# hoivb612/neural

Hardware: AMD Instinct MI355X
Metric: decode tokens/sec + prefill TFLOPS, Llama-2-7B int4-g128 at 1/2/4/8 MI355X (higher is better)
Workload: dtype f16; 1 GPU; Llama-2-7B int4-g128 sym decode linear stack, M=1 (32 x [QKV, O, gate/up+SiLU*mul, down] + lm_head), fp32 activations; group_size=128, batch=1, tp=1, parallelism=tp1, hip_graph=True

## Files before the change

neural_amd/csrc/woq_gemv.hip:

```cpp
#include <hip/hip_runtime.h>

#include <climits>
#include <cstdint>
#include <type_traits>

#include "woq_device.h"
#include "woq_kernels.h"

namespace nad {

#ifdef NAD_PHASE_TRACE
constexpr int kTraceSlots = 8, kTraceMaxWg = 16384;
__device__ unsigned long long nad_trace_buf[kTraceSlots][kTraceMaxWg];
#define NAD_TRACE(slot)                                                                       \
  do {                                                                                        \
    if (threadIdx.x == 0 && blockIdx.x < kTraceMaxWg) nad_trace_buf[slot][blockIdx.x] = wall_clock64(); \
  } while (0)
#define NAD_TRACE_MAX(slot)                                                                               \
  do {                                                                                                    \
    if ((threadIdx.x & 63) == 0 && blockIdx.x < kTraceMaxWg)                                              \
      atomicMax(&nad_trace_buf[slot][blockIdx.x], (unsigned long long)wall_clock64());                    \
  } while (0)
#else
#define NAD_TRACE(slot) \
// ... 153 lines not shown

template <int ST>
__device__ __forceinline__ float scale_to_f32(uint32_t x, int st, int sh) {
  if constexpr (ST < 0) return scale_bits_to_f32(x, st, sh);
  else if constexpr (ST == kScaleF32) return __uint_as_float(x);
  else if constexpr (ST == kScaleBF16) return __uint_as_float((x >> sh) << 16);
  else return f16_bits_to_f32(uint16_t(x >> sh));
}

constexpr int k_tile(int bits) { return bits == 4 ? 128 : (bits == 2 ? 256 : 64); }
constexpr int zp_bias(int bits) { return bits == 4 ? 8 : (bits == 2 ? 2 : 128); }

template <int BITS>
__device__ __forceinline__ Dq4 dq4_consts(uint32_t mask, uint32_t magic) {
  Dq4 q;
  q.m0 = __builtin_amdgcn_readfirstlane(mask);
  q.m1 = q.m0 << 4;
  q.mag = __builtin_amdgcn_readfirstlane(magic);
  q.s16 = splat(1.f / 16.f);
  q.c0 = splat(-(1024.f + zp_bias(BITS)));
  q.c1 = splat(-(64.f + zp_bias(BITS)));
  return q;
}

template <int BITS, bool ASYM>
__device__ __forceinline__ h8_t dequant_tile_step(const u4_t& b, int d, int zp, const Dq4& dq) {
  if constexpr (BITS == 4) {
    if constexpr (ASYM) {
      const float z = float(zp);
      return dequant4(b[d], dq, dq.c0 - splat(z), dq.c1 - splat(z));
    } else {
      return dequant4(b[d], dq, dq.c0, dq.c1);
    }
  } else {
    return BITS == 2 ? dequant2_step(b, d, zp_bias(BITS) + zp) : dequant_step<BITS>(b, d, zp_const(zp_bias(BITS) + zp));
  }
}

template <int BITS, int GPT, bool ASYM, int KSN, int ST, bool LO, class TileOff>
__device__ __forceinline__ void stage_mac(const StageRegs<GPT, KSN>& S, const Dq4& dq, const char* ab, const char* abl,
                                          TileOff tile_off, int scale_t, int ssh, f4_t& acc) {
  constexpr int SPT = k_tile(BITS) / 32, SPG = SPT / GPT;
  f4_t accg[KSN];
#pragma unroll
  for (int d = 0; d < SPT; d++) {
    const int g = GPT == 1 ? 0 : d / SPG;
#pragma unroll
    for (int i = 0; i < KSN; i++) {
      const h8_t bf = dequant_tile_step<BITS, ASYM>(S.b[i], d, S.zp[i][g], dq);
      const h8_t af = *reinterpret_cast<const h8_t*>(ab + tile_off(i) + d * 64);
      accg[i] = __builtin_amdgcn_mfma_f32_16x16x32_f16(af, bf, d % SPG == 0 ? f4_t{0.f, 0.f, 0.f, 0.f} : accg[i], 0, 0, 0);
      if constexpr (LO) {
        const h8_t afl = *reinterpret_cast<const h8_t*>(abl + tile_off(i) + d * 64);
        accg[i] = __builtin_amdgcn_mfma_f32_16x16x32_f16(afl, bf, accg[i], 0, 0, 0);
      }
    }
    if ((d + 1) % SPG == 0) {
#pragma unroll
      for (int i = 0; i < KSN; i++) acc += accg[i] * scale_to_f32<ST>(S.sc[i][g], scale_t, ssh);
    }
  }
}

__device__ __forceinline__ float reduce_slots(const float* ps, int nwl) {
  float t[16];
#pragma unroll
  for (int w = 0; w < 16; w++) t[w] = ps[min(w, nwl - 1)];
  const int full = nwl & ~3;
  float s0 = 0.f, s1 = 0.f, s2 = 0.f, s3 = 0.f;
#pragma unroll
  for (int w = 0; w < 16; w += 4)
    if (w < full) {
      s0 += t[w];
      s1 += t[w + 1];
      s2 += t[w + 2];
      s3 += t[w + 3];
    }
#pragma unroll
  for (int w = 0; w < 16; w++)
    if (w >= full && w < nwl) s0 += t[w];
  return (s0 + s1) + (s2 + s3);
}

__device__ __forceinline__ float reduce16(const float* col) {
  const float4* ps = reinterpret_cast<const float4*>(col);
  const float4 t0 = ps[0], t1 = ps[1], t2 = ps[2], t3 = ps[3];
  const float s0 = ((t0.x + t1.x) + t2.x) + t3.x, s1 = ((t0.y + t1.y) + t2.y) + t3.y;
  const float s2 = ((t0.z + t1.z) + t2.z) + t3.z, s3 = ((t0.w + t1.w) + t2.w) + t3.w;
  return (s0 + s1) + (s2 + s3);
}

__device__ __forceinline__ void unit_to_f32(int act_t, uint4 x0, uint4 x1, float (&f)[8]) {
  const uint32_t w[8] = {x0.x, x0.y, x0.z, x0.w, x1.x, x1.y, x1.z, x1.w};
  if (act_t == kActF32) {
#pragma unroll
    for (int j = 0; j < 8; j++) f[j] = __uint_as_float(w[j]);
  } else if (act_t == kActBF16) {
#pragma unroll
    for (int j = 0; j < 4; j++) {
      f[2 * j] = __uint_as_float(w[j] << 16);
      f[2 * j + 1] = __uint_as_float(w[j] & 0xFFFF0000u);
    }
  } else {
#pragma unroll
    for (int j = 0; j < 4; j++) {
      const h2_t h = as_h2(w[j]);
      f[2 * j] = float(h[0]);
      f[2 * j + 1] = float(h[1]);
    }
  }
}

template <int HILO>
__device__ __forceinline__ void unit_store(char* smem, const float (&f)[8], int row, int k, int M, int Kp) {
  h8_t hi, lo;
#pragma unroll
  for (int j = 0; j < 8; j++) {
    hi[j] = _Float16(f[j]);
    lo[j] = _Float16(f[j] - float(hi[j]));
  }
  *reinterpret_cast<h8_t*>(smem + (size_t(row) * Kp + k) * 2) = hi;
  if constexpr (HILO != 0) *reinterpret_cast<h8_t*>(smem + (size_t(M + row) * Kp + k) * 2) = lo;
}

template <int HILO>
__device__ __forceinline__ void stage_a_slow(const GemvArgs& a, char* smem, int units, int Kp) {
  for (int u = threadIdx.x; u < units; u += blockDim.x) {
    const int row = u / (Kp >> 3), k = (u - row * (Kp >> 3)) * 8;
    float f[8];
    for (int j = 0; j < 8; j++) {
      const int kk = k + j;
      f[j] = 0.f;
      if (kk < a.K) {
        const size_t src = size_t(row) * a.lda + (a.shuffle ? a.shuffle[kk] : kk);
        if (a.act_t == kActF32)
          f[j] = static_cast<const float*>(a.A)[src];
        else if (a.act_t == kActBF16)
          f[j] = bf16_bits_to_f32(static_cast<const uint16_t*>(a.A)[src]);
        else
          f[j] = float(static_cast<const _Float16*>(a.A)[src]);
      }
    }
    unit_store<HILO>(smem, f, row, k, a.M, Kp);
  }
}

template <int GPT>
constexpr int gemv_max_threads() {
  return GPT == 1 ? 1024 : 512;
}

template <int BITS, int HILO, int GPT, bool ASYM, int NST>
__global__ __launch_bounds__(gemv_max_threads<GPT>()) void woq_gemv_kernel(GemvArgs a) {
  extern __shared__ __attribute__((aligned(16))) char smem[];
  constexpr int KT = k_tile(BITS);
  static_assert(KT / 32 % GPT == 0, "groups must tile the K tile");
  const int lane = threadIdx.x & 63;
  const int wave = __builtin_amdgcn_readfirstlane(int(threadIdx.x >> 6));
  const int NW = __builtin_amdgcn_readfirstlane(int(blockDim.x >> 6));
  const int M = a.M, nt = a.nt, Kp = nt * KT;
  const int R = HILO == 0 ? M : 2 * M;
  const int nsl = (nt + KS - 1) / KS;
  NAD_TRACE(0);

  const int G = gridDim.x, bid = blockIdx.x;
  const int u0 = int(unsigned(bid) * unsigned(a.units) / unsigned(G));
  const int u1 = int(unsigned(bid + 1) * unsigned(a.units) / unsigned(G));
  const int vpu = a.dual ? 2 : 1;
  const int v0 = u0 * vpu, nv = (u1 - u0) * vpu;
  const bool idle = wave >= nsl;
  float* part = reinterpret_cast<float*>(smem + a.part_off);
// ... 141 lines not shown
    float v = y[0];
    switch (a.epi) {
      case kEpiBias:
        v += a.w[0].bias[size_t(mm) * a.w[0].bias_ld + n];
        break;
      case kEpiAddGelu:
        v = gelu_f(v + a.w[0].bias[size_t(mm) * a.w[0].bias_ld + n]);
        break;
      case kEpiGelu:
        v = gelu_f(v);
        break;
      case kEpiSilu:
        v = silu_f(v);
        break;
      case kEpiResAdd:
        v += a.res[size_t(mm) * a.ld_res + n];
        break;
      case kEpiSiluMul: {
        const float t1 = silu_f(y[0]);
        if (a.aux) a.aux[size_t(mm) * a.ld_aux + n] = t1;
        v = t1 * y[1];
        break;
      }
      case kEpiGeluMul: {
        const float t1 = gelu_f(y[0]);
        if (a.aux) a.aux[size_t(mm) * a.ld_aux + n] = t1;
        v = t1 * y[1];
        break;
      }
      default:
        break;
    }
    out[size_t(mm) * ldo + n] = v;
  }
  NAD_TRACE(3);
}

constexpr int lean_row_bytes(int bits, int ks) { return ks * (bits == 4 ? 128 : 256) * 2; }
constexpr int lean_wave_lds(int bits, int ks, int spw) { return lean_row_bytes(bits, ks) * (1 + 2 * spw); }
static int lean_ks(const GemvArgs& a) { return a.lean_ks == 1 || a.lean_ks == 2 ? a.lean_ks : KS; }
template <int GPT, int KSN>
constexpr int m1_max_threads() {
  return GPT == 1 || KSN <= 2 ? 1024 : 512;
}
static int lean_spw(const GemvArgs& a) { return a.lean_spw == 4 ? 4 : (a.lean_spw == 1 ? 1 : 2); }

static bool lean_ok(const GemvArgs& a, int bits, int waves) {
  int tpg = 0;
  const int ks = lean_ks(a);
  const int nsl = (a.nt + ks - 1) / ks;
  const int gpt = gemv_groups_per_tile(bits, a.nt, a.ng, a.bs, &tpg);
  const bool inst = bits == 4 ? (gpt == 1 || gpt == 2) : (bits == 2 && (gpt == 1 || gpt == 2 || (gpt == 4 && !a.asym)));
  return a.lean && a.M == 1 && inst && a.a_fast && nsl <= waves * lean_spw(a);
}

#ifndef NAD_M1_BATCH_NST
#define NAD_M1_BATCH_NST 3
#endif
#ifndef NAD_M1_DUAL_NST
#define NAD_M1_DUAL_NST 2
#endif

struct M1General {
  using Args = GemvArgs;
  static __device__ __forceinline__ __amdgpu_buffer_rsrc_t act_rsrc(const Args& a, int esz) { return rsrc(a.A, a.K * esz); }
  static __device__ __forceinline__ bool act_live(const Args& a, int q, int nsl, int k) { return q < nsl && k < a.K; }
  template <bool ASYM>
  static __device__ __forceinline__ void cursor_start(const Args& a, StageCursor& c, int v0, int nv, bool idle) {
    c.s = 0;
    c.rt = rsrc(a.w[0].tiles, 0);
    c.rs = c.rt;
    c.rz = c.rt;
    if (!idle && nv > 0) cursor_stripe(a, c, v0);
  }
  template <int GPT, bool ASYM, int KSN>
  static __device__ __forceinline__ void load(const Args& a, StageRegs<GPT, KSN>& S, StageCursor& c, int nv, int nsl,
                                              int wave, int NW, int v0, int lane, int vs) {
    load_stage<GPT, ASYM, KSN>(a, S, c, nv, nsl, wave, NW, v0, lane, vs);
  }
};

template <class P, int BITS, int GPT, int AT, bool ASYM, int KSN, int SPW, int NST, int ST>
__device__ __forceinline__ void m1_stream(const typename P::Args& a, int lane, int wave, int NW, int nsl, int v0,
                                          int nv, bool idle, float* part) {
  extern __shared__ __attribute__((aligned(16))) char smem[];
  constexpr int KT = k_tile(BITS);
  constexpr int RB = lean_row_bytes(BITS, KSN);
  constexpr int UNITS = KSN * KT / 8;
  constexpr int UPL = UNITS >= 64 ? UNITS / 64 : 1;
  constexpr bool PART = UNITS < 64;
  constexpr int ESZ = AT == kActF32 ? 4 : 2;
  constexpr bool HL = AT != kActF16;
  const bool ulane = !PART || lane < UNITS;

  const auto ra = P::act_rsrc(a, ESZ);
  uint4 x[SPW * UPL][2];
#pragma unroll
  for (int j = 0; j < SPW * UPL; j++) {
    const int q = wave + (j / UPL) * NW, k = q * (KSN * KT) + ((j % UPL) * 64 + lane) * 8;
    const int off = (ulane && P::act_live(a, q, nsl, k)) ? k * ESZ : kOOB;
    x[j][0] = __builtin_bit_cast(uint4, __builtin_amdgcn_raw_buffer_load_b128(ra, off, 0, 0));
    if constexpr (ESZ == 4) x[j][1] = __builtin_bit_cast(uint4, __builtin_amdgcn_raw_buffer_load_b128(ra, off + 16, 0, 0));
  }
  const int vs = a.scale_t == kScaleF32 ? (lane & 15) * 4 : (lane & 14) * 2;
  StageCursor lc;
  lc.j = idle ? nv : 0;
  lc.q = wave;
  P::template cursor_start<ASYM>(a, lc, v0, nv, idle);
  StageRegs<GPT, KSN> S[NST];
  P::template load<GPT, ASYM, KSN>(a, S[0], lc, nv, nsl, wave, NW, v0, lane, vs);
  NAD_TRACE(4);

  char* wrow = smem + wave * lean_wave_lds(BITS, KSN, SPW);
#pragma unroll
  for (int u = 0; u < UPL; u++)
    if (ulane) *reinterpret_cast<uint4*>(wrow + (u * 64 + lane) * 16) = make_uint4(0u, 0u, 0u, 0u);
#pragma unroll
  for (int j = 0; j < SPW * UPL; j++) {
    if (!ulane) break;
    h8_t hi, lo;
    if constexpr (AT == kActF16) {
      hi = __builtin_bit_cast(h8_t, x[j][0]);
    } else {
      float f[8];
      unit_to_f32(AT, x[j][0], x[j][1], f);
#pragma unroll
      for (int e = 0; e < 8; e++) {
        hi[e] = _Float16(f[e]);
        lo[e] = _Float16(f[e] - float(hi[e]));
      }
    }
    char* row = wrow + RB + (j / UPL) * 2 * RB + ((j % UPL) * 64 + lane) * 16;
    *reinterpret_cast<h8_t*>(row) = hi;
    if constexpr (HL) *reinterpret_cast<h8_t*>(row + RB) = lo;
  }
#pragma unroll
  for (int i = 1; i < NST; i++) P::template load<GPT, ASYM, KSN>(a, S[i], lc, nv, nsl, wave, NW, v0, lane, vs);
  NAD_TRACE(1);

  const int m = lane & 15, kq = lane >> 4;
  const bool isrow = m == 0 || (HL && m == 8);
  const char* abase = wrow + (isrow ? (m == 0 ? RB : 2 * RB) : 0) + kq * 16;
  const int slice_step = isrow ? 2 * RB : 0;
  const int ssh = a.scale_t == kScaleF32 ? 0 : (lane & 1) * 16;
  const Dq4 dq = dq4_consts<BITS>(a.dq_mask, a.dq_magic);

  f4_t acc = {0.f, 0.f, 0.f, 0.f};
  int cj = idle ? nv : 0, cq = wave, cs = 0;

  auto compute_stage = [&](const StageRegs<GPT, KSN>& S) {
    if (cj >= nv) return;
    const char* ab = abase + cs * slice_step;
    stage_mac<BITS, GPT, ASYM, KSN, ST, false>(S, dq, ab, ab, [](int i) { return i * KT * 2; }, a.scale_t, ssh, acc);
    cq += NW;
    cs++;
    if (cq >= nsl) {
      float r = acc[0];
      if constexpr (HL) {
        r += __shfl_down(r, 32, 64);
      }
      if (lane < 16) part[(size_t(cj) * 16 + lane) * NW + wave] = r;
      acc = f4_t{0.f, 0.f, 0.f, 0.f};
      cq = wave;
      cs = 0;
      cj++;
    }
  };

  while (cj < nv) {
#pragma unroll
    for (int i = 0; i < NST; i++) {
      compute_stage(S[i]);
      P::template load<GPT, ASYM, KSN>(a, S[i], lc, nv, nsl, wave, NW, v0, lane, vs);
    }
  }
  NAD_TRACE_MAX(2);
  __syncthreads();
}

template <int BITS, int GPT, int AT, bool ASYM, int KSN, int SPW, bool BATCH, int NST, int ST = -1>
__device__ __forceinline__ void m1_body(GemvArgs& a, int bid) {
  extern __shared__ __attribute__((aligned(16))) char smem[];
  const int lane = threadIdx.x & 63;
  const int wave = __builtin_amdgcn_readfirstlane(int(threadIdx.x >> 6));
  const int NW = __builtin_amdgcn_readfirstlane(int(blockDim.x >> 6));
  const int nsl = (a.nt + KSN - 1) / KSN;
  NAD_TRACE(0);
  if constexpr (BATCH) {
    const int p = bid / a.batch_wpp;
    bid -= p * a.batch_wpp;
    const GemvBatchEnt e = a.batch[p];
    a.A = e.act;
    a.w[0].tiles = e.tiles;
    a.w[0].scales = e.scales;
    a.w[0].zps = e.zps;
    a.w[0].out = e.out;
  }
  const int u0 = bid * a.u_q + min(bid, a.u_r);
  const int u1 = u0 + a.u_q + (bid < a.u_r ? 1 : 0);
  const int vpu = a.dual ? 2 : 1;
  const int v0 = u0 * vpu, nv = (u1 - u0) * vpu;
  float* part = reinterpret_cast<float*>(smem + a.part_off);
  m1_stream<M1General, BITS, GPT, AT, ASYM, KSN, SPW, NST, ST>(a, lane, wave, NW, nsl, v0, nv, wave >= nsl, part);

  const int nout = (u1 - u0) * 16;
  const int nwl = min(NW, nsl);
  auto emit = [&](int p, int nn, const float (&y)[2]) {
    int wsel, s;
    vstripe(a, v0 + p * vpu, wsel, s);
    if (a.dual) wsel = 0;
    const int n = s * 16 + nn;
    if (n >= sel3(wsel, a.w[0].n, a.w[1].n, a.w[2].n)) return;
    float* out = sel3(wsel, a.w[0].out, a.w[1].out, a.w[2].out);
    float v = y[0];
    switch (a.epi) {
      case kEpiBias:
        v += a.w[0].bias[n];
        break;
      case kEpiAddGelu:
        v = gelu_f(v + a.w[0].bias[n]);
        break;
      case kEpiGelu:
        v = gelu_f(v);
        break;
      case kEpiSilu:
        v = silu_f(v);
        break;
      case kEpiResAdd:
        v += a.res[n];
        break;
      case kEpiSiluMul: {
        const float t1 = silu_f(y[0]);
        if (a.aux) a.aux[n] = t1;
        v = t1 * y[1];
        break;
      }
      case kEpiGeluMul: {
        const float t1 = gelu_f(y[0]);
        if (a.aux) a.aux[n] = t1;
        v = t1 * y[1];
        break;
      }
      default:
        break;
    }
    out[n] = v;
  };
  if (nwl == 16 && NW == 16) {
    for (int o = threadIdx.x; o < nout; o += blockDim.x) {
      const int p = o >> 4, nn = o & 15;
      float y[2] = {0.f, 0.f};
#pragma unroll
      for (int h = 0; h < 2; h++)
        if (h < vpu) y[h] = reduce16(part + (size_t(p * vpu + h) * 16 + nn) * 16);
      emit(p, nn, y);
    }
    NAD_TRACE(3);
    return;
  }
  for (int o = threadIdx.x; o < nout; o += blockDim.x) {
    const int p = o >> 4, nn = o & 15;
    float y[2] = {0.f, 0.f};
#pragma unroll
    for (int h = 0; h < 2; h++)
      if (h < vpu) y[h] = reduce_slots(part + (size_t(p * vpu + h) * 16 + nn) * NW, nwl);
    emit(p, nn, y);
  }
  NAD_TRACE(3);
}

template <int BITS, int GPT, int AT, bool ASYM, int KSN, int SPW, bool BATCH, int NST, int ST>
__global__ __launch_bounds__((m1_max_threads<GPT, KSN>())) void woq_gemv_m1_kernel(GemvArgs a) {
  m1_body<BITS, GPT, AT, ASYM, KSN, SPW, BATCH, NST, ST>(a, int(blockIdx.x));
}

template <int B1, int G1, int K1, int B2, int G2, int K2, int AT>
__global__ __launch_bounds__(1024) void woq_gemv_m1_dual_kernel(GemvArgs a, GemvArgs b, int ga) {
  if (int(blockIdx.x) < ga)
    m1_body<B1, G1, AT, false, K1, 1, false, NAD_M1_DUAL_NST>(a, int(blockIdx.x));
  else
    m1_body<B2, G2, AT, false, K2, 1, false, NAD_M1_DUAL_NST>(b, int(blockIdx.x) - ga);
}

template <int NWT>
struct M1Sel {
  int w, s;
  __device__ __forceinline__ M1Sel(const GemvM1Args<NWT>& a, int v) {
    if constexpr (NWT == 1) {
      w = 0;
      s = v;
    } else if constexpr (NWT == 2) {
      w = v & 1;
      s = v >> 1;
    } else {
      w = (v >= a.sb1 ? 1 : 0) + (v >= a.sb2 ? 1 : 0);
      s = v - (w == 0 ? 0 : (w == 1 ? a.sb1 : a.sb2));
    }
  }
};
template <int NWT, class T>
__device__ __forceinline__ T m1_pick(int w, const T (&x)[3]) {
  if constexpr (NWT == 1) return x[0];
  else if constexpr (NWT == 2) return w == 0 ? x[0] : x[1];
  else return sel3(w, x[0], x[1], x[2]);
}
#define NAD_M1_FIELD(args, wi, f) \
  m1_pick<NWT>(wi, {args.w[0].f, args.w[NWT > 1 ? 1 : 0].f, args.w[NWT > 2 ? 2 : 0].f})

template <int NWT, bool ASYM>
__device__ __forceinline__ void m1s_cursor_stripe(const GemvM1Args<NWT>& a, StageCursor& c, int v, bool on) {
  const M1Sel<NWT> vs(a, v);
  c.s = vs.s;
  const void* const tp[3] = {a.w[0].tiles, a.w[NWT > 1 ? 1 : 0].tiles, a.w[NWT > 2 ? 2 : 0].tiles};
  const void* const sp[3] = {a.w[0].scales, a.w[NWT > 1 ? 1 : 0].scales, a.w[NWT > 2 ? 2 : 0].scales};
  const int tb[3] = {a.w[0].tiles_bytes, a.w[NWT > 1 ? 1 : 0].tiles_bytes, a.w[NWT > 2 ? 2 : 0].tiles_bytes};
  const int sb[3] = {a.w[0].scales_bytes, a.w[NWT > 1 ? 1 : 0].scales_bytes, a.w[NWT > 2 ? 2 : 0].scales_bytes};
  c.rt = rsrc(m1_pick<NWT>(vs.w, tp), on ? m1_pick<NWT>(vs.w, tb) : 0);
  c.rs = rsrc(m1_pick<NWT>(vs.w, sp), on ? m1_pick<NWT>(vs.w, sb) : 0);
  if constexpr (ASYM) {
    const void* const zp[3] = {a.w[0].zps, a.w[NWT > 1 ? 1 : 0].zps, a.w[NWT > 2 ? 2 : 0].zps};
    const int zb[3] = {a.w[0].zps_bytes, a.w[NWT > 1 ? 1 : 0].zps_bytes, a.w[NWT > 2 ? 2 : 0].zps_bytes};
    c.rz = rsrc(m1_pick<NWT>(vs.w, zp), on ? m1_pick<NWT>(vs.w, zb) : 0);
  } else {
    c.rz = c.rs;
  }
}

template <int GPT, bool ASYM, int KSN, int NWT>
__device__ __forceinline__ void m1s_load_stage(const GemvM1Args<NWT>& a, StageRegs<GPT, KSN>& S, StageCursor& c, int nv,
                                               int nsl, int wave, int NW, int v0, int lane, int vs) {
  const bool on = c.j < nv;
  stage_loads<ASYM>(a, S, c, on, lane, vs);
  if (on) {
    c.q += NW;
    if (c.q >= nsl) {
      c.q = wave;
      c.j++;
      m1s_cursor_stripe<NWT, ASYM>(a, c, v0 + c.j, c.j < nv);
    }
  }
}

template <int NWT>
struct M1Spec {
  using Args = GemvM1Args<NWT>;
  static __device__ __forceinline__ __amdgpu_buffer_rsrc_t act_rsrc(const Args& a, int) { return rsrc(a.A, a.a_bytes); }
  static __device__ __forceinline__ bool act_live(const Args&, int, int, int) { return true; }
  template <bool ASYM>
  static __device__ __forceinline__ void cursor_start(const Args& a, StageCursor& c, int v0, int nv, bool) {
    m1s_cursor_stripe<NWT, ASYM>(a, c, v0, c.j < nv);
  }
  template <int GPT, bool ASYM, int KSN>
  static __device__ __forceinline__ void load(const Args& a, StageRegs<GPT, KSN>& S, StageCursor& c, int nv, int nsl,
                                              int wave, int NW, int v0, int lane, int vs) {
    m1s_load_stage<GPT, ASYM, KSN, NWT>(a, S, c, nv, nsl, wave, NW, v0, lane, vs);
  }
};

template <int BITS, int GPT, int AT, bool ASYM, int KSN, int SPW, int NST, int ST, int NWT, bool L16>
__global__ __launch_bounds__((m1_max_threads<GPT, KSN>())) void woq_gemv_m1s_kernel(GemvM1Args<NWT> a) {
  extern __shared__ __attribute__((aligned(16))) char smem[];
  static_assert(NWT >= 1 && NWT <= 3, "1 weight, the {gate, up} pair, or 3 weights");
  constexpr int VPU = NWT == 2 ? 2 : 1;
  const int lane = threadIdx.x & 63;
  const int wave = __builtin_amdgcn_readfirstlane(int(threadIdx.x >> 6));
  const int NW = L16 ? 16 : a.nw;
  const int nsl = a.nsl;
  NAD_TRACE(0);
  const int bid = int(blockIdx.x);
  const int u0 = bid * a.u_q + min(bid, a.u_r);
  const int nu = a.u_q + (bid < a.u_r ? 1 : 0);
  const int v0 = u0 * VPU, nv = nu * VPU;
  const bool idle = !L16 && wave >= nsl;
  float* part = reinterpret_cast<float*>(smem + a.part_off);
  m1_stream<M1Spec<NWT>, BITS, GPT, AT, ASYM, KSN, SPW, NST, ST>(a, lane, wave, NW, nsl, v0, nv, idle, part);

  const int nout = nu * 16;
  for (int o = threadIdx.x; o < nout; o += NW * 64) {
    const int p = o >> 4, nn = o & 15;
    float y[VPU];
#pragma unroll
    for (int h = 0; h < VPU; h++) {
      if constexpr (L16)
        y[h] = reduce16(part + (size_t(p * VPU + h) * 16 + nn) * 16);
      else
        y[h] = reduce_slots(part + (size_t(p * VPU + h) * 16 + nn) * NW, min(NW, nsl));
    }
    const M1Sel<NWT> vsel(a, v0 + p * VPU);
    const int wsel = NWT == 2 ? 0 : vsel.w;
    const int n = vsel.s * 16 + nn;
    if (n >= NAD_M1_FIELD(a, wsel, n)) continue;
    float* out = NAD_M1_FIELD(a, wsel, out);
    if constexpr (NWT == 2) {
      const float t1 = silu_f(y[0]);
      if (a.aux) a.aux[n] = t1;
      out[n] = t1 * y[VPU - 1];
    } else {
      out[n] = y[0];
    }
  }
  NAD_TRACE(3);
}

template <auto K, class... Args>
static hipError_t launch_big_lds(dim3 g, dim3 b, size_t lds, hipStream_t st, const Args&... args) {
  static bool attr_set = false;
  if (!attr_set) {
    hipError_t e = hipFuncSetAttribute(reinterpret_cast<const void*>(K), hipFuncAttributeMaxDynamicSharedMemorySize,
                                       160 * 1024);
    if (e != hipSuccess) return e;
    attr_set = true;
  }
  hipLaunchKernelGGL(K, g, b, lds, st, args...);
  return hipGetLastError();
}

static int m1_stages_per_wave(const GemvArgs& a, int ksn, int waves) {
  const int nsl = (a.nt + ksn - 1) / ksn;
  return (a.u_q + (a.u_r ? 1 : 0)) * (a.dual ? 2 : 1) * ((nsl + waves - 1) / waves);
}
static int m1_nst(const GemvArgs& a, int ksn, int waves) {
  if (a.m1_nst == 1 || a.m1_nst == 2) return a.m1_nst;
  const int spw = m1_stages_per_wave(a, ksn, waves);
  return spw >= 7 || (ksn == 1 && spw >= 4) ? 2 : 1;
}

template <int V>
using IntC = std::integral_constant<int, V>;
template <class F>
static auto by_act(const GemvArgs& a, F f) {
  if (a.act_t == kActF32) return f(IntC<kActF32>{});
  if (a.act_t == kActF16) return f(IntC<kActF16>{});
  return f(IntC<kActBF16>{});
}
template <class F>
static auto by_asym(const GemvArgs& a, F f) {
  return a.asym ? f(std::true_type{}) : f(std::false_type{});
}

template <int BITS, int HILO, int GPT, bool ASYM>
static hipError_t gemv_launch4(const GemvArgs& a, dim3 g, dim3 b, size_t lds, hipStream_t st) {
  const int spw = m1_stages_per_wave(a, KS, int(b.x / 64));
  const int nst = a.m1_nst == 1 ? 1 : (a.m1_nst == 3 ? 3 : (spw <= 2 ? 1 : 3));
  return nst == 1 ? launch_big_lds<woq_gemv_kernel<BITS, HILO, GPT, ASYM, 1>>(g, b, lds, st, a)
                  : launch_big_lds<woq_gemv_kernel<BITS, HILO, GPT, ASYM, 3>>(g, b, lds, st, a);
}

template <int BITS, int GPT, int AT, bool ASYM, int KSN, int SPW, int ST>
static hipError_t gemv_m1_launch5(const GemvArgs& a, dim3 g, dim3 b, size_t lds, hipStream_t st) {
  if (a.batch)
    return launch_big_lds<woq_gemv_m1_kernel<BITS, GPT, AT, ASYM, KSN, SPW, true, NAD_M1_BATCH_NST, ST>>(g, b, lds, st, a);
  return m1_nst(a, KSN, int(b.x / 64)) == 1
             ? launch_big_lds<woq_gemv_m1_kernel<BITS, GPT, AT, ASYM, KSN, SPW, false, 1, ST>>(g, b, lds, st, a)
             : launch_big_lds<woq_gemv_m1_kernel<BITS, GPT, AT, ASYM, KSN, SPW, false, 2, ST>>(g, b, lds, st, a);
}
#ifndef NAD_INT2_ST
#define NAD_INT2_ST 1
#endif
template <int BITS, int GPT, int AT, bool ASYM, int ST = -1>
static hipError_t gemv_m1_launch4(const GemvArgs& a, dim3 g, dim3 b, size_t lds, hipStream_t st) {
  if constexpr (BITS == 2 && ST < 0 && NAD_INT2_ST) {
    if (a.scale_t == kScaleF32) return gemv_m1_launch4<BITS, GPT, AT, ASYM, kScaleF32>(a, g, b, lds, st);
    if (a.scale_t == kScaleBF16) return gemv_m1_launch4<BITS, GPT, AT, ASYM, kScaleBF16>(a, g, b, lds, st);
    return gemv_m1_launch4<BITS, GPT, AT, ASYM, kScaleF16>(a, g, b, lds, st);
  } else {
    if (a.lean_ks == 1) return gemv_m1_launch5<BITS, GPT, AT, ASYM, 1, 1, ST>(a, g, b, lds, st);
    if (a.lean_ks == 2) return gemv_m1_launch5<BITS, GPT, AT, ASYM, 2, 1, ST>(a, g, b, lds, st);
    return a.lean_spw == 4 ? gemv_m1_launch5<BITS, GPT, AT, ASYM, KS, 4, ST>(a, g, b, lds, st)
                           : gemv_m1_launch5<BITS, GPT, AT, ASYM, KS, 2, ST>(a, g, b, lds, st);
  }
}
template <int NWT>
static GemvM1Args<NWT> m1s_args(const GemvArgs& a, int ksn, int waves) {
  GemvM1Args<NWT> c{};
  const int esz = a.act_t == kActF32 ? 4 : 2, ssz = a.scale_t == kScaleF32 ? 4 : 2;
  c.A = a.A;
  c.a_bytes = a.K * esz;
  c.nsl = (a.nt + ksn - 1) / ksn;
  c.u_q = a.u_q;
  c.u_r = a.u_r;
  c.nt = a.nt;
  c.ng = a.ng;
  c.tpg_shift = a.tpg_shift;
  c.scale_t = a.scale_t;
  c.nw = waves;
  c.part_off = a.part_off;
  c.dq_mask = a.dq_mask;
  c.dq_magic = a.dq_magic;
  c.sb1 = a.stripe_base[1];
  c.sb2 = a.stripe_base[2];
  for (int i = 0; i < NWT; i++) {
    const SkinnyWeight& w = a.w[i];
    c.w[i].tiles = w.tiles;
    c.w[i].scales = w.scales;
    c.w[i].zps = w.zps;
    c.w[i].tiles_bytes = w.ns * a.nt * 1024;
    c.w[i].scales_bytes = w.ns * a.ng * 16 * ssz;
    c.w[i].zps_bytes = w.ns * a.ng * 16;
    c.w[i].n = w.n;
    c.w[i].out = w.out;
  }
  c.aux = a.aux;
  return c;
}
template <int BITS, int GPT, int AT, bool ASYM, int KSN, int SPW, int NST, int ST, int NWT, bool L16>
static hipError_t m1s_go(const GemvArgs& a, dim3 g, dim3 b, size_t lds, hipStream_t st) {
  return launch_big_lds<woq_gemv_m1s_kernel<BITS, GPT, AT, ASYM, KSN, SPW, NST, ST, NWT, L16>>(
      g, b, lds, st, m1s_args<NWT>(a, KSN, int(b.x / 64)));
}
static int m1s_nwt(const GemvArgs& a) {
  if (a.batch || !a.m1_spec) return 0;
  if (a.dual) return a.epi == kEpiSiluMul ? 2 : 0;
  if (a.epi != kEpiNone) return 0;
  const int nw = 1 + (a.stripe_base[1] != INT_MAX ? 1 : 0) + (a.stripe_base[2] != INT_MAX ? 1 : 0);
  return nw == 1 || nw == 3 ? nw : 0;
}
template <int BITS, int GPT, int AT, bool ASYM, int ST>
static bool m1s_launch3(const GemvArgs& a, dim3 g, dim3 b, size_t lds, hipStream_t st, hipError_t* e) {
  const int nwt = m1s_nwt(a), waves = int(b.x / 64), ks = lean_ks(a);
  if (nwt == 0) return false;
  const int nsl = (a.nt + ks - 1) / ks;
  const bool l16 = waves == 16 && nsl >= 16;
  const int nst = m1_nst(a, ks, waves);
#define NAD_M1S(KSN, SPW, NST, NWT, L16)                                                         \
  do {                                                                                           \
    if (e) *e = m1s_go<BITS, GPT, AT, ASYM, KSN, SPW, NST, ST, NWT, L16>(a, g, b, lds, st);      \
    return true;                                                                                 \
  } while (0)
#define NAD_M1S_NARROW(KSN)                               \
  do {                                                    \
    if (nst == 1) {                                       \
      if (nwt == 1 && l16) NAD_M1S(KSN, 1, 1, 1, true);   \
      if (nwt == 1) NAD_M1S(KSN, 1, 1, 1, false);         \
      if (nwt == 2 && l16) NAD_M1S(KSN, 1, 1, 2, true);   \
      if (nwt == 2) NAD_M1S(KSN, 1, 1, 2, false);         \
      if (nwt == 3 && l16) NAD_M1S(KSN, 1, 1, 3, true);   \
      if (nwt == 3) NAD_M1S(KSN, 1, 1, 3, false);         \
    } else if (nwt == 1) {                                \
      if (l16) NAD_M1S(KSN, 1, 2, 1, true);               \
      NAD_M1S(KSN, 1, 2, 1, false);                       \
    }                                                     \
    return false;                                         \
  } while (0)
  if (ks == 1) NAD_M1S_NARROW(1);
  if (ks == 2) NAD_M1S_NARROW(2);
  if (l16 || (GPT != 1 && waves > 8)) return false;
  if (lean_spw(a) == 4) {
    if (nwt == 1 && nst == 1) NAD_M1S(KS, 4, 1, 1, false);
    return false;
  }
  if (nst == 1) {
    if (nwt == 1) NAD_M1S(KS, 2, 1, 1, false);
    if (nwt == 2) NAD_M1S(KS, 2, 1, 2, false);
    NAD_M1S(KS, 2, 1, 3, false);
  }
  if (nwt == 1) NAD_M1S(KS, 2, 2, 1, false);
  return false;
#undef NAD_M1S_NARROW
#undef NAD_M1S
}
#if !defined(GEMV_PART) || GEMV_PART == 2
bool gemv_m1s_launch_b4(const GemvArgs& a, int gpt, dim3 g, dim3 b, size_t lds, hipStream_t st, hipError_t* e) {
  if (gpt == 1)
    return by_act(a, [&](auto at) {
      return by_asym(a, [&](auto as) { return m1s_launch3<4, 1, at.value, as.value, -1>(a, g, b, lds, st, e); });
    });
  if (gpt == 2 && a.act_t == kActF32)
    return by_asym(a, [&](auto as) { return m1s_launch3<4, 2, kActF32, as.value, -1>(a, g, b, lds, st, e); });
  return false;
}
#else
bool gemv_m1s_launch_b4(const GemvArgs& a, int gpt, dim3 g, dim3 b, size_t lds, hipStream_t st, hipError_t* e);
#endif
#if !defined(GEMV_PART) || GEMV_PART == 3
template <int GPT>
static bool m1s_launch_b2g(const GemvArgs& a, dim3 g, dim3 b, size_t lds, hipStream_t st, hipError_t* e) {
  if (a.scale_t == kScaleF32) return m1s_launch3<2, GPT, kActF32, false, NAD_INT2_ST ? kScaleF32 : -1>(a, g, b, lds, st, e);
  if (a.scale_t == kScaleBF16) return m1s_launch3<2, GPT, kActF32, false, NAD_INT2_ST ? kScaleBF16 : -1>(a, g, b, lds, st, e);
  return m1s_launch3<2, GPT, kActF32, false, NAD_INT2_ST ? kScaleF16 : -1>(a, g, b, lds, st, e);
}
bool gemv_m1s_launch_b2(const GemvArgs& a, int gpt, dim3 g, dim3 b, size_t lds, hipStream_t st, hipError_t* e) {
  if (a.asym || a.act_t != kActF32) return false;
  if (gpt == 1) return m1s_launch_b2g<1>(a, g, b, lds, st, e);
  if (gpt == 2) return m1s_launch_b2g<2>(a, g, b, lds, st, e);
  if (gpt == 4) return m1s_launch_b2g<4>(a, g, b, lds, st, e);
  return false;
}
#else
bool gemv_m1s_launch_b2(const GemvArgs& a, int gpt, dim3 g, dim3 b, size_t lds, hipStream_t st, hipError_t* e);
#endif

template <int BITS, int GPT>
static hipError_t gemv_m1_launch2(const GemvArgs& a, dim3 g, dim3 b, size_t lds, hipStream_t st) {
  return by_act(a, [&](auto at) {
    return by_asym(a, [&](auto as) { return gemv_m1_launch4<BITS, GPT, at.value, as.value>(a, g, b, lds, st); });
  });
}
#if !defined(GEMV_PART) || GEMV_PART == 1
hipError_t gemv_m1_launch_b2(const GemvArgs& a, int gpt, dim3 g, dim3 b, size_t lds, hipStream_t st) {
  if (gpt == 1) return gemv_m1_launch2<2, 1>(a, g, b, lds, st);
  if (gpt == 2) return gemv_m1_launch2<2, 2>(a, g, b, lds, st);
  if (gpt == 4 && !a.asym)
    return by_act(a, [&](auto at) { return gemv_m1_launch4<2, 4, at.value, false>(a, g, b, lds, st); });
  return hipErrorInvalidValue;
}
#else
hipError_t gemv_m1_launch_b2(const GemvArgs& a, int gpt, dim3 g, dim3 b, size_t lds, hipStream_t st);
#endif
#if !defined(GEMV_PART) || GEMV_PART == 0
static hipError_t gemv_m1_launch(const GemvArgs& a, int bits, int gpt, dim3 g, dim3 b, size_t lds, hipStream_t st) {
  if (bits == 4) {
    if (gpt == 1) return gemv_m1_launch2<4, 1>(a, g, b, lds, st);
    if (gpt == 2) return gemv_m1_launch2<4, 2>(a, g, b, lds, st);
    return hipErrorInvalidValue;
  }
  return gemv_m1_launch_b2(a, gpt, g, b, lds, st);
}

template <int BITS, int HILO>
static hipError_t gemv_launch2(const GemvArgs& a, int gpt, dim3 g, dim3 b, size_t lds, hipStream_t st) {
  constexpr int SPT = k_tile(BITS) / 32;
  return by_asym(a, [&](auto as) {
    if (gpt == 1) return gemv_launch4<BITS, HILO, 1, as.value>(a, g, b, lds, st);
    if (gpt == 2) return gemv_launch4<BITS, HILO, 2, as.value>(a, g, b, lds, st);
    if constexpr (SPT % 4 == 0) {
      if (gpt == 4) return gemv_launch4<BITS, HILO, 4, as.value>(a, g, b, lds, st);
    }
    return hipError_t(hipErrorInvalidValue);
  });
}

template <int BITS>
static hipError_t gemv_launch1(const GemvArgs& a, int hilo, int gpt, dim3 g, dim3 b, size_t lds, hipStream_t st) {
  if (hilo == 0) return gemv_launch2<BITS, 0>(a, gpt, g, b, lds, st);
  if (hilo == 1) return gemv_launch2<BITS, 1>(a, gpt, g, b, lds, st);
  return gemv_launch2<BITS, 2>(a, gpt, g, b, lds, st);
}

size_t gemv_lds_layout(GemvArgs& a, int bits, int waves, int grid) {
  if (lean_ok(a, bits, waves)) {
    const int upw = (a.units + grid - 1) / grid;
    a.part_off = waves * lean_wave_lds(bits, lean_ks(a), lean_spw(a));
    return size_t(a.part_off) + size_t(upw) * (a.dual ? 2 : 1) * waves * 16 * 4;
  }
  const int KT = bits == 4 ? 128 : (bits == 2 ? 256 : 64);
  const int R = a.act_t == kActF16 ? a.M : 2 * a.M;
  const size_t kp = size_t(a.nt) * KT;
  const size_t abytes = (size_t(R) + 1) * kp * 2;
  const int upw = (a.units + grid - 1) / grid;
  const size_t nv = size_t(upw) * (a.dual ? 2 : 1);
  a.part_off = int((abytes + 15) & ~size_t(15));
  return size_t(a.part_off) + nv * waves * a.M * 16 * 4;
}

int gemv_waves(int bits, int nt, int ng, int bs) {
  int tpg = 0;
  const int gpt = gemv_groups_per_tile(bits, nt, ng, bs, &tpg);
  const int maxw = gpt > 1 ? 8 : 16;
  const int nsl = (nt + KS - 1) / KS;
  const int spw = (nsl + maxw - 1) / maxw;
  return (nsl + spw - 1) / spw;
}

void gemv_lean_slices(GemvArgs& a, int bits, int* waves, int ks_pref) {
  a.lean_ks = KS;
  a.lean_spw = 2;
  if (a.M == 1 && a.lean && (a.nt + KS - 1) / KS > 2 * *waves) {
    a.lean_spw = 4;
    if (!lean_ok(a, bits, *waves)) a.lean_spw = 2;
    return;
  }
  if ((ks_pref != 2 && ks_pref != 3) || a.M != 1 || !a.lean) return;
  const int ks = a.nt <= 16 && ks_pref == 2 ? 1 : 2;
  const int nsl = (a.nt + ks - 1) / ks;
  if (nsl > 16 || nsl <= *waves) return;
  if (!lean_ok(a, bits, *waves)) return;
  a.lean_ks = ks;
  a.lean_spw = 1;
  if (!lean_ok(a, bits, nsl)) {
    a.lean_ks = KS;
    a.lean_spw = 2;
    return;
  }
  *waves = nsl;
}

int gemv_groups_per_tile(int bits, int nt, int ng, int bs, int* tpg) {
  const int KT = bits == 4 ? 128 : (bits == 2 ? 256 : 64);
  if (ng == 1) {
    *tpg = 0;
    return 1;
  }
  if (bs % KT == 0) {
    *tpg = bs / KT;
    return (*tpg & (*tpg - 1)) == 0 ? 1 : 0;
  }
  if (KT % bs == 0 && bs % 32 == 0) {
    *tpg = 1;
    const int g = KT / bs;
    return (g == 2 || g == 4) ? g : 0;
  }
  return 0;
}

bool gemv_uses_m1(const GemvArgs& a, int bits, int waves) { return lean_ok(a, bits, waves); }

bool gemv_uses_m1s(const GemvArgs& a, int bits, int waves) {
  int tpg = 0;
  const int gpt = gemv_groups_per_tile(bits, a.nt, a.ng, a.bs, &tpg);
  if (!lean_ok(a, bits, waves)) return false;
  return bits == 4 ? gemv_m1s_launch_b4(a, gpt, dim3(1), dim3(waves * 64), 0, nullptr, nullptr)
                   : gemv_m1s_launch_b2(a, gpt, dim3(1), dim3(waves * 64), 0, nullptr, nullptr);
}

bool gemv_dual_ok(const GemvArgs& a, int bits_a, const GemvArgs& b, int bits_b, int waves) {
  int tpg = 0;
  const int ga = gemv_groups_per_tile(bits_a, a.nt, a.ng, a.bs, &tpg), gb = gemv_groups_per_tile(bits_b, b.nt, b.ng, b.bs, &tpg);
  const bool pair = bits_a == 2 && bits_b == 4 && ((ga == 4 && gb == 2) || (ga == 2 && gb == 1));
  return pair && !a.asym && !b.asym && a.lean_ks == 1 && b.lean_ks == 2 && a.act_t == kActF32 && b.act_t == kActF32 &&
         waves == 16 && lean_ok(a, bits_a, waves) && lean_ok(b, bits_b, waves);
}

hipError_t launch_gemv_dual(const GemvArgs& a, const GemvArgs& b, int ga, int gb, int waves, size_t lds,
                            hipStream_t stream) {
  int tpg = 0;
  const int g1 = gemv_groups_per_tile(2, a.nt, a.ng, a.bs, &tpg);
// ... 57 lines not shown
```

neural_amd/csrc/woq_kernels.h:

```cpp
#pragma once
#include <hip/hip_runtime.h>

#include <algorithm>
#include <cstdint>

#include "woq_layout.h"

namespace nad {

enum ActType : int { kActF32 = 0, kActF16 = 1, kActBF16 = 2 };

struct RepackArgs {
  const uint8_t* src_q;
  const void* src_s;
  const int8_t* src_z;
  int ntile, packrow, kpad, cstep;
  int src_bits;
  uint64_t nel;
  int raw;
  int src_e8m0;
  int bits, n, k, ns, nt, ng, scale_t, kmajor;
  uint32_t* dst_tiles;
  void* dst_scales;
  int8_t* dst_zps;
// ... 23 lines not shown
  int scale_t;
  int epi;
  int vec_ok;
  int a_fast;
  const float* res;
  int ld_res;
  float* aux;
  int ld_aux;
  SkinnyWeight w[3];
};

struct GemmArgs {
  const void* A;
  int lda, M, K;
  int scale_t;
  int epi;
  int vec_ok;
  const float* res;
  int ld_res;
  const float* aux;
  int ld_aux;
  int stagger;
  int fold;
  int ksw;
  int ksplit;
  int ktiles;
  float* part;
  int ldp;
  _Float16* out16;
  int ldo16;
  const _Float16* aux16;
  int tpg_shift;
  int xcd_sg;
  int xcd_w;
  int nwt;
  int nbn_cut[2];
  int nbn_all;
  SkinnyWeight wf[2];
  int xcd_tile;
  SkinnyWeight w;
};

struct GemvBatchEnt {
  const void* act;
  const void* tiles;
  const void* scales;
  const int8_t* zps;
  float* out;
  const void* pad[3];
};

struct GemvArgs {
  const void* A;
  int lda, M, K;
  int act_t;
  int dual;
  int units;
  int stripe_base[3];
  int nt, ng, bs;
  int tpg_shift;
  int scale_t;
  int asym;
  int epi;
  int a_fast;
  const int32_t* shuffle;
  const float* res;
  int ld_res;
  float* aux;
  int ld_aux;
  int part_off;
  uint32_t dq_mask;
  uint32_t dq_magic;
  int u_q, u_r;
  int lean;
  int lean_ks;
  int lean_spw;
  SkinnyWeight w[3];
  const GemvBatchEnt* batch;
  int batch_wpp;
  int m1_nst;
  int m1_spec;
};

struct GemvM1Weight {
  const void* tiles;
  const void* scales;
  const int8_t* zps;
  int tiles_bytes, scales_bytes, zps_bytes;
  int n;
  float* out;
};
template <int NWS>
struct GemvM1Args {
  const void* A;
  int a_bytes;
  int nsl;
  int u_q, u_r;
  int nt, ng;
  int tpg_shift;
  int scale_t;
  int nw;
  int part_off;
  uint32_t dq_mask, dq_magic;
  int sb1, sb2;
  GemvM1Weight w[NWS];
  float* aux;
};

hipError_t launch_repack(const RepackArgs& a, hipStream_t stream);
hipError_t launch_skinny(const SkinnyArgs& a, int bits, int act_t, int waves_per_wg, int stripes, int ch,
                         hipStream_t stream);
hipError_t launch_gemm(const GemmArgs& a, int bits, int act_t, hipStream_t stream);
hipError_t launch_gemm2(const GemmArgs& a, const _Float16* A16, int lda16, hipStream_t stream);
hipError_t launch_gemm3(const GemmArgs& a, const _Float16* A16, int lda16, hipStream_t stream);
int gemm4_mode(int bits, int blocksize, int ng, int kpad, bool asym);

struct QuantU8Args {
  const void* A;
  int lda, M, K, bs, ng;
  const int32_t* shuffle;
  int8_t* aq;
  int ldq, kp;
  float2* sa;
  uint8_t* q_u8;
  int ldu;
  float* s_out;
  uint8_t* z_out;
  float* red_out;
  int ld_scale;
};
struct I8Args {
  const int8_t* aq;
  int ldq;
  int a_signed;
  const float2* sa;
  int M, K;
  const uint16_t* red;
  int red_ld;
  int scale_t;
  int epi;
  const float* res;
  int ld_res;
  const float* aux;
  int ld_aux;
  SkinnyWeight w;
};
struct Q80Args {
  const void* A;
  int lda, M, K;
  int8_t* aq;
  int ldq, kp;
  float2* sa;
  int8_t* blocks;
};
typedef Q80Args Q81Args;
struct MinTermArgs {
  const void* A;
  int lda, M, K;
  int a_vec;
  const float* S;
  int s_ld, s_st;
  const uint16_t* mins;
  const uint16_t* scales;
  float qbias;
  int ns, ng, kmajor;
  GemmArgs g;
// ... 51 lines not shown
```

Before: 1032 tokens/s.

## Pack m1s kernel args into scalars and specialise fixed wave-count reductions

The specialized M=1 GEMV kernel now takes its hot fields (activation, first two weights' tiles/scales, packed geometry words) as direct scalar kernel arguments and rebuilds the argument struct on device. The aim is to shrink or reorder the kernarg payload so the fields needed first land in early SGPRs. The boolean L16 template is generalised to a compile-time slot count NSC, adding fixed-size reductions for 7 and 11 waves with padded partial-sum stride. LDS sizing is rounded up to match the padding. Phase-trace instrumentation is also added under an ifdef. The change adds bit-packing limits with a fallback path when fields do not fit.

Result: faster. 1051 tokens/s (median of 6 runs) (+1.8%).

```diff
diff --git a/neural_amd/csrc/woq_gemv.hip b/neural_amd/csrc/woq_gemv.hip
--- a/neural_amd/csrc/woq_gemv.hip
+++ b/neural_amd/csrc/woq_gemv.hip
@@ -259,11 +259,25 @@
   return (s0 + s1) + (s2 + s3);
 }
 
-__device__ __forceinline__ float reduce16(const float* col) {
+template <int N>
+__device__ __forceinline__ float reduce_fixed(const float* col) {
+  static_assert(N >= 4 && N <= 16, "at least one whole group of four");
+  constexpr int NV = (N + 3) / 4, FULL = N / 4;
   const float4* ps = reinterpret_cast<const float4*>(col);
-  const float4 t0 = ps[0], t1 = ps[1], t2 = ps[2], t3 = ps[3];
-  const float s0 = ((t0.x + t1.x) + t2.x) + t3.x, s1 = ((t0.y + t1.y) + t2.y) + t3.y;
-  const float s2 = ((t0.z + t1.z) + t2.z) + t3.z, s3 = ((t0.w + t1.w) + t2.w) + t3.w;
+  float4 t[NV];
+#pragma unroll
+  for (int i = 0; i < NV; i++) t[i] = ps[i];
+  float s0 = t[0].x, s1 = t[0].y, s2 = t[0].z, s3 = t[0].w;
+#pragma unroll
+  for (int i = 1; i < FULL; i++) {
+    s0 += t[i].x;
+    s1 += t[i].y;
+    s2 += t[i].z;
+    s3 += t[i].w;
+  }
+  if constexpr (N % 4 > 0) s0 += t[FULL].x;
+  if constexpr (N % 4 > 1) s0 += t[FULL].y;
+  if constexpr (N % 4 > 2) s0 += t[FULL].z;
   return (s0 + s1) + (s2 + s3);
 }
 
@@ -571,7 +585,7 @@
 
 template <class P, int BITS, int GPT, int AT, bool ASYM, int KSN, int SPW, int NST, int ST>
 __device__ __forceinline__ void m1_stream(const typename P::Args& a, int lane, int wave, int NW, int nsl, int v0,
-                                          int nv, bool idle, float* part) {
+                                          int nv, bool idle, float* part, int PS) {
   extern __shared__ __attribute__((aligned(16))) char smem[];
   constexpr int KT = k_tile(BITS);
   constexpr int RB = lean_row_bytes(BITS, KSN);
@@ -637,10 +651,27 @@
   f4_t acc = {0.f, 0.f, 0.f, 0.f};
   int cj = idle ? nv : 0, cq = wave, cs = 0;
 
+#ifdef NAD_PHASE_TRACE
+  unsigned long long tr_first = 0, tr_later = 0, tr_k = 0;
+#endif
   auto compute_stage = [&](const StageRegs<GPT, KSN>& S) {
     if (cj >= nv) return;
     const char* ab = abase + cs * slice_step;
+#ifdef NAD_PHASE_TRACE
+    asm volatile("s_waitcnt vmcnt(0)" ::: "memory");
+    const unsigned long long tr0 = wall_clock64();
+#endif
     stage_mac<BITS, GPT, ASYM, KSN, ST, false>(S, dq, ab, ab, [](int i) { return i * KT * 2; }, a.scale_t, ssh, acc);
+#ifdef NAD_PHASE_TRACE
+    {
+      const int sink = __builtin_amdgcn_readfirstlane(__float_as_int(acc[0]));
+      asm volatile("" ::"s"(sink));
+      const unsigned long long d = wall_clock64() - tr0;
+      if (tr_k == 0) tr_first = d;
+      else tr_later += d;
+      tr_k++;
+    }
+#endif
     cq += NW;
     cs++;
     if (cq >= nsl) {
@@ -648,7 +679,7 @@
       if constexpr (HL) {
         r += __shfl_down(r, 32, 64);
       }
-      if (lane < 16) part[(size_t(cj) * 16 + lane) * NW + wave] = r;
+      if (lane < 16) part[(size_t(cj) * 16 + lane) * PS + wave] = r;
       acc = f4_t{0.f, 0.f, 0.f, 0.f};
       cq = wave;
       cs = 0;
@@ -663,6 +694,13 @@
       P::template load<GPT, ASYM, KSN>(a, S[i], lc, nv, nsl, wave, NW, v0, lane, vs);
     }
   }
+#ifdef NAD_PHASE_TRACE
+  if (threadIdx.x == 0 && blockIdx.x < kTraceMaxWg) {
+    nad_trace_buf[5][blockIdx.x] = tr_first;
+    nad_trace_buf[6][blockIdx.x] = tr_later;
+    nad_trace_buf[7][blockIdx.x] = tr_k;
+  }
+#endif
   NAD_TRACE_MAX(2);
   __syncthreads();
 }
@@ -690,7 +728,7 @@
   const int vpu = a.dual ? 2 : 1;
   const int v0 = u0 * vpu, nv = (u1 - u0) * vpu;
   float* part = reinterpret_cast<float*>(smem + a.part_off);
-  m1_stream<M1General, BITS, GPT, AT, ASYM, KSN, SPW, NST, ST>(a, lane, wave, NW, nsl, v0, nv, wave >= nsl, part);
+  m1_stream<M1General, BITS, GPT, AT, ASYM, KSN, SPW, NST, ST>(a, lane, wave, NW, nsl, v0, nv, wave >= nsl, part, NW);
 
   const int nout = (u1 - u0) * 16;
   const int nwl = min(NW, nsl);
@@ -741,7 +779,7 @@
       float y[2] = {0.f, 0.f};
 #pragma unroll
       for (int h = 0; h < 2; h++)
-        if (h < vpu) y[h] = reduce16(part + (size_t(p * vpu + h) * 16 + nn) * 16);
+        if (h < vpu) y[h] = reduce_fixed<16>(part + (size_t(p * vpu + h) * 16 + nn) * 16);
       emit(p, nn, y);
     }
     NAD_TRACE(3);
@@ -846,23 +884,56 @@
   }
 };
 
-template <int BITS, int GPT, int AT, bool ASYM, int KSN, int SPW, int NST, int ST, int NWT, bool L16>
-__global__ __launch_bounds__((m1_max_threads<GPT, KSN>())) void woq_gemv_m1s_kernel(GemvM1Args<NWT> a) {
+template <int BITS, int GPT, int AT, bool ASYM, int KSN, int SPW, int NST, int ST, int NWT, int NSC>
+__global__ __launch_bounds__((m1_max_threads<GPT, KSN>())) void woq_gemv_m1s_kernel(
+    const void* A, const void* tiles0, const void* scales0, const void* tiles1, const void* scales1, int a_bytes,
+    uint32_t uqr, uint32_t geom, int ns0, GemvM1Rest<NWT> r) {
   extern __shared__ __attribute__((aligned(16))) char smem[];
   static_assert(NWT >= 1 && NWT <= 3, "1 weight, the {gate, up} pair, or 3 weights");
+  static_assert(NSC == 0 || (NSC >= 4 && NSC <= 16), "slots per column: 0 = by the launch");
   constexpr int VPU = NWT == 2 ? 2 : 1;
+  GemvM1Args<NWT> a;
+  a.A = A;
+  a.a_bytes = a_bytes;
+  a.u_q = int(uqr & 0xFFFFu);
+  a.u_r = int(uqr >> 16);
+  a.nt = int(geom & ((1u << kM1GeomNgShift) - 1));
+  a.ng = int((geom >> kM1GeomNgShift) & ((1u << (kM1GeomTpgShift - kM1GeomNgShift)) - 1));
+  a.tpg_shift = int((geom >> kM1GeomTpgShift) & 31u);
+  a.scale_t = int((geom >> kM1GeomScaleShift) & 3u);
+  a.nw = int(geom >> kM1GeomWavesShift);
+  a.nsl = (a.nt + KSN - 1) / KSN;
+  a.part_off = r.part_off;
+  a.dq_mask = r.dq_mask;
+  a.dq_magic = r.dq_magic;
+  a.sb1 = r.sb1;
+  a.sb2 = r.sb2;
+  a.aux = r.aux;
+#pragma unroll
+  for (int i = 0; i < NWT; i++) {
+    const int ns = i == 0 || NWT == 2 ? ns0 : r.ns[i];
+    a.w[i].tiles = i == 0 ? tiles0 : (i == 1 ? tiles1 : r.tiles2);
+    a.w[i].scales = i == 0 ? scales0 : (i == 1 ? scales1 : r.scales2);
+    a.w[i].zps = r.zps[i];
+    a.w[i].tiles_bytes = (ns * a.nt) << 10;
+    a.w[i].scales_bytes = (ns * a.ng) << (a.scale_t == kScaleF32 ? 6 : 5);
+    a.w[i].zps_bytes = (ns * a.ng) << 4;
+    a.w[i].n = r.n[i];
+    a.w[i].out = r.out[i];
+  }
   const int lane = threadIdx.x & 63;
   const int wave = __builtin_amdgcn_readfirstlane(int(threadIdx.x >> 6));
-  const int NW = L16 ? 16 : a.nw;
+  const int NW = NSC ? NSC : a.nw;
+  const int PS = NSC ? (NSC + 3) & ~3 : NW;
   const int nsl = a.nsl;
   NAD_TRACE(0);
   const int bid = int(blockIdx.x);
   const int u0 = bid * a.u_q + min(bid, a.u_r);
   const int nu = a.u_q + (bid < a.u_r ? 1 : 0);
   const int v0 = u0 * VPU, nv = nu * VPU;
-  const bool idle = !L16 && wave >= nsl;
+  const bool idle = NSC == 0 && wave >= nsl;
   float* part = reinterpret_cast<float*>(smem + a.part_off);
-  m1_stream<M1Spec<NWT>, BITS, GPT, AT, ASYM, KSN, SPW, NST, ST>(a, lane, wave, NW, nsl, v0, nv, idle, part);
+  m1_stream<M1Spec<NWT>, BITS, GPT, AT, ASYM, KSN, SPW, NST, ST>(a, lane, wave, NW, nsl, v0, nv, idle, part, PS);
 
   const int nout = nu * 16;
   for (int o = threadIdx.x; o < nout; o += NW * 64) {
@@ -870,8 +941,8 @@
     float y[VPU];
 #pragma unroll
     for (int h = 0; h < VPU; h++) {
-      if constexpr (L16)
-        y[h] = reduce16(part + (size_t(p * VPU + h) * 16 + nn) * 16);
+      if constexpr (NSC != 0)
+        y[h] = reduce_fixed<NSC>(part + (size_t(p * VPU + h) * 16 + nn) * PS);
       else
         y[h] = reduce_slots(part + (size_t(p * VPU + h) * 16 + nn) * NW, min(NW, nsl));
     }
@@ -960,19 +1031,8 @@
   }
 }
 template <int NWT>
-static GemvM1Args<NWT> m1s_args(const GemvArgs& a, int ksn, int waves) {
-  GemvM1Args<NWT> c{};
-  const int esz = a.act_t == kActF32 ? 4 : 2, ssz = a.scale_t == kScaleF32 ? 4 : 2;
-  c.A = a.A;
-  c.a_bytes = a.K * esz;
-  c.nsl = (a.nt + ksn - 1) / ksn;
-  c.u_q = a.u_q;
-  c.u_r = a.u_r;
-  c.nt = a.nt;
-  c.ng = a.ng;
-  c.tpg_shift = a.tpg_shift;
-  c.scale_t = a.scale_t;
-  c.nw = waves;
+static GemvM1Rest<NWT> m1s_rest(const GemvArgs& a) {
+  GemvM1Rest<NWT> c{};
   c.part_off = a.part_off;
   c.dq_mask = a.dq_mask;
   c.dq_magic = a.dq_magic;
@@ -980,54 +1040,67 @@
   c.sb2 = a.stripe_base[2];
   for (int i = 0; i < NWT; i++) {
     const SkinnyWeight& w = a.w[i];
-    c.w[i].tiles = w.tiles;
-    c.w[i].scales = w.scales;
-    c.w[i].zps = w.zps;
-    c.w[i].tiles_bytes = w.ns * a.nt * 1024;
-    c.w[i].scales_bytes = w.ns * a.ng * 16 * ssz;
-    c.w[i].zps_bytes = w.ns * a.ng * 16;
-    c.w[i].n = w.n;
-    c.w[i].out = w.out;
-  }
+    c.ns[i] = w.ns;
+    c.zps[i] = w.zps;
+    c.n[i] = w.n;
+    c.out[i] = w.out;
+  }
+  c.tiles2 = NWT > 2 ? a.w[2].tiles : nullptr;
+  c.scales2 = NWT > 2 ? a.w[2].scales : nullptr;
   c.aux = a.aux;
   return c;
 }
-template <int BITS, int GPT, int AT, bool ASYM, int KSN, int SPW, int NST, int ST, int NWT, bool L16>
+static bool m1s_packable(const GemvArgs& a, int nwt, int waves) {
+  if (a.u_q < 0 || a.u_q > 0xFFFF || a.u_r < 0 || a.u_r > 0xFFFF) return false;
+  if (a.nt >= (1 << kM1GeomNgShift) || a.ng >= (1 << (kM1GeomTpgShift - kM1GeomNgShift))) return false;
+  if (a.tpg_shift < 0 || a.tpg_shift > 31 || a.scale_t < 0 || a.scale_t > 3 || waves > 16) return false;
+  return nwt != 2 || a.w[0].ns == a.w[1].ns;
+}
+template <int BITS, int GPT, int AT, bool ASYM, int KSN, int SPW, int NST, int ST, int NWT, int NSC>
 static hipError_t m1s_go(const GemvArgs& a, dim3 g, dim3 b, size_t lds, hipStream_t st) {
-  return launch_big_lds<woq_gemv_m1s_kernel<BITS, GPT, AT, ASYM, KSN, SPW, NST, ST, NWT, L16>>(
-      g, b, lds, st, m1s_args<NWT>(a, KSN, int(b.x / 64)));
-}
-static int m1s_nwt(const GemvArgs& a) {
+  const int esz = a.act_t == kActF32 ? 4 : 2;
+  const uint32_t uqr = uint32_t(a.u_q) | uint32_t(a.u_r) << 16;
+  const uint32_t geom = uint32_t(a.nt) | uint32_t(a.ng) << kM1GeomNgShift | uint32_t(a.tpg_shift) << kM1GeomTpgShift |
+                        uint32_t(a.scale_t) << kM1GeomScaleShift | uint32_t(b.x / 64) << kM1GeomWavesShift;
+  return launch_big_lds<woq_gemv_m1s_kernel<BITS, GPT, AT, ASYM, KSN, SPW, NST, ST, NWT, NSC>>(
+      g, b, lds, st, a.A, a.w[0].tiles, a.w[0].scales, NWT > 1 ? a.w[1].tiles : nullptr,
+      NWT > 1 ? a.w[1].scales : nullptr, a.K * esz, uqr, geom, a.w[0].ns, m1s_rest<NWT>(a));
+}
+static int m1s_nwt(const GemvArgs& a, int waves) {
   if (a.batch || !a.m1_spec) return 0;
-  if (a.dual) return a.epi == kEpiSiluMul ? 2 : 0;
-  if (a.epi != kEpiNone) return 0;
-  const int nw = 1 + (a.stripe_base[1] != INT_MAX ? 1 : 0) + (a.stripe_base[2] != INT_MAX ? 1 : 0);
-  return nw == 1 || nw == 3 ? nw : 0;
+  int nwt = 0;
+  if (a.dual) {
+    nwt = a.epi == kEpiSiluMul ? 2 : 0;
+  } else if (a.epi == kEpiNone) {
+    const int nw = 1 + (a.stripe_base[1] != INT_MAX ? 1 : 0) + (a.stripe_base[2] != INT_MAX ? 1 : 0);
+    nwt = nw == 1 || nw == 3 ? nw : 0;
+  }
+  return nwt != 0 && m1s_packable(a, nwt, waves) ? nwt : 0;
 }
 template <int BITS, int GPT, int AT, bool ASYM, int ST>
 static bool m1s_launch3(const GemvArgs& a, dim3 g, dim3 b, size_t lds, hipStream_t st, hipError_t* e) {
-  const int nwt = m1s_nwt(a), waves = int(b.x / 64), ks = lean_ks(a);
+  const int waves = int(b.x / 64), ks = lean_ks(a), nwt = m1s_nwt(a, waves);
   if (nwt == 0) return false;
   const int nsl = (a.nt + ks - 1) / ks;
   const bool l16 = waves == 16 && nsl >= 16;
   const int nst = m1_nst(a, ks, waves);
-#define NAD_M1S(KSN, SPW, NST, NWT, L16)                                                         \
+#define NAD_M1S(KSN, SPW, NST, NWT, NSC)                                                         \
   do {                                                                                           \
-    if (e) *e = m1s_go<BITS, GPT, AT, ASYM, KSN, SPW, NST, ST, NWT, L16>(a, g, b, lds, st);      \
+    if (e) *e = m1s_go<BITS, GPT, AT, ASYM, KSN, SPW, NST, ST, NWT, NSC>(a, g, b, lds, st);      \
     return true;                                                                                 \
   } while (0)
 #define NAD_M1S_NARROW(KSN)                               \
   do {                                                    \
     if (nst == 1) {                                       \
-      if (nwt == 1 && l16) NAD_M1S(KSN, 1, 1, 1, true);   \
-      if (nwt == 1) NAD_M1S(KSN, 1, 1, 1, false);         \
-      if (nwt == 2 && l16) NAD_M1S(KSN, 1, 1, 2, true);   \
-      if (nwt == 2) NAD_M1S(KSN, 1, 1, 2, false);         \
-      if (nwt == 3 && l16) NAD_M1S(KSN, 1, 1, 3, true);   \
-      if (nwt == 3) NAD_M1S(KSN, 1, 1, 3, false);         \
+      if (nwt == 1 && l16) NAD_M1S(KSN, 1, 1, 1, 16);     \
+      if (nwt == 1) NAD_M1S(KSN, 1, 1, 1, 0);             \
+      if (nwt == 2 && l16) NAD_M1S(KSN, 1, 1, 2, 16);     \
+      if (nwt == 2) NAD_M1S(KSN, 1, 1, 2, 0);             \
+      if (nwt == 3 && l16) NAD_M1S(KSN, 1, 1, 3, 16);     \
+      if (nwt == 3) NAD_M1S(KSN, 1, 1, 3, 0);             \
     } else if (nwt == 1) {                                \
-      if (l16) NAD_M1S(KSN, 1, 2, 1, true);               \
-      NAD_M1S(KSN, 1, 2, 1, false);                       \
+      if (l16) NAD_M1S(KSN, 1, 2, 1, 16);                 \
+      NAD_M1S(KSN, 1, 2, 1, 0);                           \
     }                                                     \
     return false;                                         \
   } while (0)
@@ -1035,15 +1108,19 @@
   if (ks == 2) NAD_M1S_NARROW(2);
   if (l16 || (GPT != 1 && waves > 8)) return false;
   if (lean_spw(a) == 4) {
-    if (nwt == 1 && nst == 1) NAD_M1S(KS, 4, 1, 1, false);
+    if (nwt == 1 && nst == 1 && waves == 7 && nsl >= 7) NAD_M1S(KS, 4, 1, 1, 7);
+    if (nwt == 1 && nst == 1) NAD_M1S(KS, 4, 1, 1, 0);
     return false;
   }
   if (nst == 1) {
-    if (nwt == 1) NAD_M1S(KS, 2, 1, 1, false);
-    if (nwt == 2) NAD_M1S(KS, 2, 1, 2, false);
-    NAD_M1S(KS, 2, 1, 3, false);
-  }
-  if (nwt == 1) NAD_M1S(KS, 2, 2, 1, false);
+    if constexpr (GPT == 1) {
+      if (nwt == 1 && waves == 11 && nsl >= 11) NAD_M1S(KS, 2, 1, 1, 11);
+    }
+    if (nwt == 1) NAD_M1S(KS, 2, 1, 1, 0);
+    if (nwt == 2) NAD_M1S(KS, 2, 1, 2, 0);
+    NAD_M1S(KS, 2, 1, 3, 0);
+  }
+  if (nwt == 1) NAD_M1S(KS, 2, 2, 1, 0);
   return false;
 #undef NAD_M1S_NARROW
 #undef NAD_M1S
@@ -1130,7 +1207,7 @@
   if (lean_ok(a, bits, waves)) {
     const int upw = (a.units + grid - 1) / grid;
     a.part_off = waves * lean_wave_lds(bits, lean_ks(a), lean_spw(a));
-    return size_t(a.part_off) + size_t(upw) * (a.dual ? 2 : 1) * waves * 16 * 4;
+    return size_t(a.part_off) + size_t(upw) * (a.dual ? 2 : 1) * ((waves + 3) & ~3) * 16 * 4;
   }
   const int KT = bits == 4 ? 128 : (bits == 2 ? 256 : 64);
   const int R = a.act_t == kActF16 ? a.M : 2 * a.M;
diff --git a/neural_amd/csrc/woq_kernels.h b/neural_amd/csrc/woq_kernels.h
--- a/neural_amd/csrc/woq_kernels.h
+++ b/neural_amd/csrc/woq_kernels.h
@@ -129,6 +129,20 @@
   int m1_spec;
 };
 
+constexpr int kM1GeomNgShift = 9, kM1GeomTpgShift = 20, kM1GeomScaleShift = 25, kM1GeomWavesShift = 27;
+template <int NWS>
+struct GemvM1Rest {
+  int part_off;
+  uint32_t dq_mask, dq_magic;
+  int sb1, sb2;
+  int ns[3];
+  const void* tiles2;
+  const void* scales2;
+  const int8_t* zps[NWS];
+  int n[NWS];
+  float* out[NWS];
+  float* aux;
+};
 struct GemvM1Weight {
   const void* tiles;
   const void* scales;
```
